# descriptinc/audiotools

Measured on NVIDIA H100. Metric: clips/sec (10s@44.1kHz) log-mel+LUFS pipeline, higher is better.
Workload: dtype f32

## Files before the change

### audiotools_b200/csrc/fft_warp.cuh

```cuda
#pragma once
#include "b2a_common.h"

namespace b2a {
namespace spectral {

__device__ __forceinline__ float2 rot_mi(float2 a) { return make_float2(a.y, -a.x); }

__device__ __forceinline__ float2 cadd(float2 a, float2 b) { return add2(a, b); }
__device__ __forceinline__ float2 csub(float2 a, float2 b) { return add2(a, neg2(b)); }
__device__ __forceinline__ float2 cmul(float2 a, float2 b) {
  return fma2(bcast2(a.x), b, mul2(bcast2(a.y), make_float2(-b.y, b.x)));
}

__device__ __forceinline__ constexpr float cos_pi16(int j) {
  return j == 0 ? 1.0f
       : j == 1 ? 0.98078528040323043f
       : j == 2 ? 0.92387953251128674f
       : j == 3 ? 0.83146961230254524f
       : j == 4 ? 0.70710678118654752f
       : j == 5 ? 0.55557023301960222f
       : j == 6 ? 0.38268343236508977f
       : j == 7 ? 0.19509032201612827f
       : j == 8 ? 0.0f
                : -cos_pi16(16 - j);
}

__device__ __forceinline__ constexpr float cos_pi32(int j) {
  return (j & 1) == 0 ? cos_pi16(j / 2)
       : j == 1 ? 0.99518472667219689f
       : j == 3 ? 0.95694033573220887f
       : j == 5 ? 0.88192126434835503f
       : j == 7 ? 0.77301045336273696f
       : j == 9 ? 0.63439328416364549f
       : j == 11 ? 0.47139673682599764f
       : j == 13 ? 0.29028467725446236f
       : j == 15 ? 0.09801714032956060f
                 : -cos_pi32(32 - j);
}

template <int R, int K>
__device__ __forceinline__ float2 mul_wr(float2 o) {
  constexpr int j = 32 * K / R;
  if constexpr (j == 0) {
    return o;
  } else if constexpr (j == 8) {
    return make_float2(o.y, -o.x);
  } else if constexpr (j == 4) {
    constexpr float h = 0.70710678118654752f;
    return make_float2(h * (o.x + o.y), h * (o.y - o.x));
  } else if constexpr (j == 12) {
    constexpr float h = 0.70710678118654752f;
    return make_float2(h * (o.y - o.x), -h * (o.x + o.y));
  } else {
    constexpr float c = cos_pi16(j);
    constexpr float sn = cos_pi16(j <= 8 ? 8 - j : j - 8);
    return make_float2(fmaf(o.x, c, o.y * sn), fmaf(o.y, c, -o.x * sn));
  }
}

template <int R, int S, bool PRE = false>
struct DFT {
  template <int K>
  static __device__ __forceinline__ void comb(const float2 (&e)[R / 2], const float2 (&o)[R / 2], float2* out) {
    constexpr int j = 32 * K / R;
    if constexpr (R == 2 && PRE) {
      out[K] = e[K];
      out[K + R / 2] = o[K];
    } else if constexpr (j == 0) {
      out[K] = add2(e[K], o[K]);
      out[K + R / 2] = add2(e[K], neg2(o[K]));
    } else if constexpr (j == 8) {
      out[K] = add2(e[K], rot_mi(o[K]));
      out[K + R / 2] = add2(e[K], neg2(rot_mi(o[K])));
    } else if constexpr (j == 4 || j == 12) {
      constexpr float h = 0.70710678118654752f;
      const float2 pq = add2(o[K], rot_mi(o[K]));
      float2 s;
      if constexpr (j == 4) s = fma2(bcast2(h), pq, e[K]);
      else s = fma2(make_float2(h, -h), make_float2(pq.y, pq.x), e[K]);
      out[K] = s;
      out[K + R / 2] = fma2(bcast2(2.0f), e[K], neg2(s));
    } else {
      constexpr float c = cos_pi16(j);
      constexpr float sn = cos_pi16(j <= 8 ? 8 - j : j - 8);
      const float2 s = fma2(o[K], bcast2(c), fma2(rot_mi(o[K]), bcast2(sn), e[K]));
      out[K] = s;
      out[K + R / 2] = fma2(bcast2(2.0f), e[K], neg2(s));
    }
    if constexpr (K + 1 < R / 2) comb<K + 1>(e, o, out);
  }
  static __device__ __forceinline__ void run(const float2* in, float2* out) {
    float2 e[R / 2], o[R / 2];
    DFT<R / 2, 2 * S, PRE>::run(in, e);
    DFT<R / 2, 2 * S, PRE>::run(in + S, o);
    comb<0>(e, o, out);
  }
};
template <int S, bool PRE>
struct DFT<1, S, PRE> {
  static __device__ __forceinline__ void run(const float2* in, float2* out) { out[0] = in[0]; }
};

template <int LOG2N>
struct WPlan {
  static constexpr int N = 1 << LOG2N;
  static constexpr int LPF = N / 32;
  static constexpr int FPW = 32 / LPF;
  static constexpr int R1 = LPF;
  static constexpr int B1 = 32 / R1;
  static constexpr int NWARP = 8;
  static constexpr int G = NWARP * FPW;
  static constexpr int FR = (G >= 16) ? G : (LOG2N == 10 ? 8 : 16);
  static constexpr bool LEAN = (LOG2N == 10);
  static constexpr int NTW = LEAN ? 10 : ((R1 >= 2) ? B1 * (R1 - 1) : 0);
  static constexpr int NUT = LEAN ? 1 : 16;
  static constexpr int XB = ((N + N / 32 + 4 + 3) / 4) * 4 + (N >= 256 ? 128 : 32);
};

__device__ __forceinline__ float fast_sqrt(float v) {
#ifdef B2A_SIM
  return sqrtf(v);
#else
  float r;
  asm("sqrt.approx.ftz.f32 %0, %1;" : "=f"(r) : "f"(v));
  return r;
#endif
}

__device__ __forceinline__ float fast_log2(float v) {
#ifdef B2A_SIM
  return log2f(v);
#else
  float r;
  asm("lg2.approx.f32 %0, %1;" : "=f"(r) : "f"(v));
  return r;
#endif
}

template <int LOG2N, bool PRE0 = false>
__device__ __forceinline__ void warp_fft(float2 (&z)[32], float* xb, const float2* tw, int l) {
  using PL = WPlan<LOG2N>;
  constexpr int LPF = PL::LPF, R1 = PL::R1, B1 = PL::B1;
  {
    float2 o[32];
    DFT<32, 1, PRE0>::run(z, o);
#pragma unroll
    for (int t = 0; t < 32; ++t) z[t] = o[t];
  }
  if constexpr (R1 >= 2) {
#pragma unroll
    for (int t = 0; t < 32; ++t) xb[l * 33 + t] = z[t].x;
    __syncwarp();
#pragma unroll
    for (int m = 0; m < 32; ++m) { const int e = l + LPF * m; z[m].x = xb[e + (e >> 5)]; }
    __syncwarp();
#pragma unroll
    for (int t = 0; t < 32; ++t) xb[l * 33 + t] = z[t].y;
    __syncwarp();
#pragma unroll
    for (int m = 0; m < 32; ++m) { const int e = l + LPF * m; z[m].y = xb[e + (e >> 5)]; }
    __syncwarp();
    if constexpr (PL::LEAN) {
      const float2 w8 = tw[7 * LPF + l], w16 = tw[8 * LPF + l], w24 = tw[9 * LPF + l];
      z[8] = cmul(z[8], w8); z[16] = cmul(z[16], w16); z[24] = cmul(z[24], w24);
#pragma unroll
      for (int b = 1; b < 8; ++b) {
        const float2 wb = tw[(b - 1) * LPF + l];
        z[b] = cmul(z[b], wb);
        z[8 + b] = cmul(cmul(z[8 + b], wb), w8);
        z[16 + b] = cmul(cmul(z[16 + b], wb), w16);
        z[24 + b] = cmul(cmul(z[24 + b], wb), w24);
      }
    }
#pragma unroll
    for (int b = 0; b < B1; ++b) {
      if constexpr (!PL::LEAN) {
#pragma unroll
        for (int t = 1; t < R1; ++t)
          z[b + B1 * t] = cmul(z[b + B1 * t], tw[(b * (R1 - 1) + (t - 1)) * LPF + l]);
      }
      float2 o[R1];
      DFT<R1, B1>::run(&z[b], o);
#pragma unroll
      for (int t = 0; t < R1; ++t) z[b + B1 * t] = o[t];
    }
  }
}

template <int LOG2N, int M>
__device__ __forceinline__ float2 untangle_twiddle(const float2* ut, float2 u0, int l) {
  using PL = WPlan<LOG2N>;
  if constexpr (PL::LEAN) {
    if constexpr (M == 0) {
      return u0;
    } else {
      constexpr float c = cos_pi32(M), sn = cos_pi32(16 - M);
      return fma2(bcast2(u0.x), make_float2(c, -sn), mul2(bcast2(u0.y), make_float2(sn, c)));
    }
  } else {
    return ut[M * PL::LPF + l];
  }
}

template <int LOG2N>
__device__ __forceinline__ float2 untangle_twiddle_m(const float2* ut, float2 u0, int l, int m) {
  switch (m) {
    case 0: return untangle_twiddle<LOG2N, 0>(ut, u0, l);
    case 1: return untangle_twiddle<LOG2N, 1>(ut, u0, l);
    case 2: return untangle_twiddle<LOG2N, 2>(ut, u0, l);
    case 3: return untangle_twiddle<LOG2N, 3>(ut, u0, l);
    case 4: return untangle_twiddle<LOG2N, 4>(ut, u0, l);
    case 5: return untangle_twiddle<LOG2N, 5>(ut, u0, l);
    case 6: return untangle_twiddle<LOG2N, 6>(ut, u0, l);
    case 7: return untangle_twiddle<LOG2N, 7>(ut, u0, l);
    case 8: return untangle_twiddle<LOG2N, 8>(ut, u0, l);
    case 9: return untangle_twiddle<LOG2N, 9>(ut, u0, l);
    case 10: return untangle_twiddle<LOG2N, 10>(ut, u0, l);
    case 11: return untangle_twiddle<LOG2N, 11>(ut, u0, l);
    case 12: return untangle_twiddle<LOG2N, 12>(ut, u0, l);
    case 13: return untangle_twiddle<LOG2N, 13>(ut, u0, l);
    case 14: return untangle_twiddle<LOG2N, 14>(ut, u0, l);
    default: return untangle_twiddle<LOG2N, 15>(ut, u0, l);
  }
}

template <int LOG2N>
__device__ __forceinline__ void untangle(const float2 (&z)[32], const float2* ut, int l, int src_lane, float2 (&a)[16],
                                         float2 (&b)[16], float2& h) {
  const float2 u0 = ut[l];
#pragma unroll
  for (int m = 0; m < 16; ++m) {
    const float2 zk = z[m];
    float2 zn;
    zn.x = __shfl_sync(0xffffffffu, z[31 - m].x, src_lane);
    zn.y = __shfl_sync(0xffffffffu, z[31 - m].y, src_lane);
    if (l == 0) zn = z[(32 - m) & 31];
    const float2 xe = add2(zk, make_float2(zn.x, -zn.y));
    const float2 xo = add2(make_float2(zk.y, -zk.x), make_float2(zn.y, zn.x));
    const float2 w = untangle_twiddle_m<LOG2N>(ut, u0, l, m);
    const float2 xk = fma2(bcast2(w.x), xo, fma2(make_float2(-w.y, w.y), make_float2(xo.y, xo.x), xe));
    const float2 d = fma2(bcast2(2.0f), xe, neg2(xk));
    a[m] = xk;
    b[m] = make_float2(d.x, -d.y);
  }
  h = make_float2(2.0f * z[16].x, -2.0f * z[16].y);
}


template <int LPF>
__device__ __forceinline__ int partner_lane(int lane) {
  return (lane & ~(LPF - 1)) | ((LPF - (lane & (LPF - 1))) & (LPF - 1));
}

template <int LOG2N>
__device__ __forceinline__ void load_frame(const float* fs, const float* win, int hop, float2 (&z)[32], int l) {
  constexpr int LPF = WPlan<LOG2N>::LPF;
  if ((hop & 1) == 0) {
#pragma unroll
    for (int m = 0; m < 16; ++m) {
      const int e0 = l + LPF * m, e1 = e0 + LPF * 16;
      const float2 s0 = *reinterpret_cast<const float2*>(fs + 2 * e0);
      const float2 w0 = *reinterpret_cast<const float2*>(win + 2 * e0);
      const float2 s1 = *reinterpret_cast<const float2*>(fs + 2 * e1);
      const float2 w1 = *reinterpret_cast<const float2*>(win + 2 * e1);
      const float2 a = mul2(s0, w0);
      z[m] = fma2(s1, w1, a);
      z[m + 16] = fma2(neg2(s1), w1, a);
    }
  } else {
#pragma unroll
    for (int m = 0; m < 16; ++m) {
      const int e0 = l + LPF * m, e1 = e0 + LPF * 16;
      const float ax = fs[2 * e0] * win[2 * e0], ay = fs[2 * e0 + 1] * win[2 * e0 + 1];
      const float sx = fs[2 * e1], sy = fs[2 * e1 + 1], wx = win[2 * e1], wy = win[2 * e1 + 1];
      z[m] = make_float2(fmaf(sx, wx, ax), fmaf(sy, wy, ay));
      z[m + 16] = make_float2(fmaf(-sx, wx, ax), fmaf(-sy, wy, ay));
    }
  }
}

template <int LOG2N, int NUT = 16>
__device__ __forceinline__ void warp_fft_tables(float2* tw, float2* ut) {
  using PL = WPlan<LOG2N>;
  constexpr int N = PL::N, LPF = PL::LPF, R1 = PL::R1;
  const int tid = threadIdx.x, nt = blockDim.x;
  for (int i = tid; i < PL::NTW * LPF; i += nt) {
    const int slot = i / LPF, ll = i - slot * LPF;
    int e;
    if constexpr (PL::LEAN) {
      e = ll * (slot < 7 ? slot + 1 : 8 * (slot - 6));
    } else {
      const int b = slot / (R1 > 1 ? R1 - 1 : 1), t = slot - b * (R1 > 1 ? R1 - 1 : 1) + 1;
      e = (ll + LPF * b) * t;
    }
    float sn, cs;
    sincospif(-2.0f * (float)e / (float)N, &sn, &cs);
    tw[i] = make_float2(cs, sn);
  }
  for (int i = tid; i < NUT * LPF; i += nt) {
    const int m = i / LPF, ll = i - m * LPF;
    float sn, cs;
    sincospif(-(float)(ll + LPF * m) / (float)N, &sn, &cs);
    ut[i] = make_float2(cs, sn);
  }
}

}
}
```

### audiotools_b200/csrc/spectral.cu

```cuda
#include "b2a_common.h"
#include "fft_warp.cuh"
#include "grad_internal.h"
#include "spectral_internal.h"

namespace b2a {
namespace spectral {

constexpr int THREADS = 256;
constexpr int E = 16;

template <int LOG2N>
struct Plan {
  static constexpr int N = 1 << LOG2N;
  static constexpr int TPF = N / E;
  static constexpr int G = THREADS / TPF;
  static constexpr int P = (LOG2N + 3) / 4;
  static constexpr int radix(int p) {
    return (p < LOG2N / 4) ? 16 : (1 << (LOG2N % 4));
  }
  static constexpr int ns(int p) { return 1 << (4 * p); }
  static constexpr int slots(int p) { return p == 0 ? 0 : (E / radix(p)) * (radix(p) - 1); }
  static constexpr int slot_off(int p) {
    int o = 0;
    for (int i = 1; i < p; ++i) o += slots(i);
    return o;
  }
  static constexpr int NSLOT = slot_off(P);
  static constexpr int BUF = N + N / 16 + 1;
  static constexpr int MAG = N + 4;
  static constexpr int FR = (G >= 16) ? G : ((LOG2N >= 11) ? 2 * G : ((LOG2N == 10) ? 4 * G : 16));
};

__device__ __forceinline__ void stage_span(const Params& p, float* sp, int row, int tile, int n0, int FR, int ws,
                                           float g) {
  const int tid = threadIdx.x, T = p.T, hop = p.hop, span = p.span;
  const float* xr = p.x + (size_t)row * (size_t)T;
  const int own_lo = n0 * hop;
  const int own_hi = (tile == p.n_tiles - 1) ? T : min(T, (n0 + FR) * hop);
  const bool interior = (ws >= 0) && (ws + span <= T);
  if (interior) {
    const float* src = xr + ws;
    const bool vec = ((((uintptr_t)src) & 15) == 0) && ((span & 3) == 0) &&
                     (!p.y_out || (((uintptr_t)(p.y_out + (size_t)row * T + ws)) & 15) == 0);
    if (vec) {
      for (int i = tid * 4; i < span; i += (int)blockDim.x * 4) {
        float4 v = *reinterpret_cast<const float4*>(src + i);
        if (p.gain) { v.x *= g; v.y *= g; v.z *= g; v.w *= g; }
        *reinterpret_cast<float4*>(sp + i) = v;
        if (p.y_out) {
          const int w = ws + i;
          if (w >= own_lo && w + 3 < own_hi) {
            *reinterpret_cast<float4*>(p.y_out + (size_t)row * T + w) = v;
          } else {
            float vv[4] = {v.x, v.y, v.z, v.w};
#pragma unroll
            for (int e = 0; e < 4; ++e)
              if (w + e >= own_lo && w + e < own_hi) p.y_out[(size_t)row * T + w + e] = vv[e];
          }
        }
      }
    } else {
      for (int i = tid; i < span; i += (int)blockDim.x) {
        float v = __ldg(src + i);
        if (p.gain) v *= g;
        sp[i] = v;
        const int w = ws + i;
        if (p.y_out && w >= own_lo && w < own_hi) p.y_out[(size_t)row * T + w] = v;
      }
    }
  } else {
    for (int i = tid; i < span; i += (int)blockDim.x) {
      const int w = ws + i;
      const int u = src_index(w, T, p.pad, p.right_pad, p.pad_mode);
      float v = (u >= 0) ? __ldg(xr + u) : 0.f;
      if (p.gain) v *= g;
      sp[i] = v;
      if (p.y_out && w >= own_lo && w < own_hi) p.y_out[(size_t)row * T + w] = v;
    }
  }
  if (p.y_out) {
    for (int w = max(own_lo, ws + span) + tid; w < own_hi; w += (int)blockDim.x) {
      float v = __ldg(xr + w);
      if (p.gain) v *= g;
      p.y_out[(size_t)row * T + w] = v;
    }
  }
}

__device__ __forceinline__ void writeback_scaled(const Params& p, const float* sp, int row, int tile, int n0, int FR,
                                                 int ws, float g) {
  const int tid = threadIdx.x, T = p.T, hop = p.hop, span = p.span;
  const int own_lo = n0 * hop;
  const int own_hi = (tile == p.n_tiles - 1) ? T : min(T, (n0 + FR) * hop);
  float* yr = p.y_out + (size_t)row * (size_t)T;
  const int lo = max(own_lo, ws), hi = min(own_hi, ws + span);
  const bool vec = (((lo - ws) & 3) == 0) && ((((uintptr_t)(yr + lo)) & 15) == 0);
  if (vec) {
    const int n4 = (hi - lo) >> 2;
    for (int i = tid; i < n4; i += (int)blockDim.x) {
      float4 v = *reinterpret_cast<const float4*>(sp + (lo - ws) + 4 * i);
      v.x *= g; v.y *= g; v.z *= g; v.w *= g;
      st_stream4(yr + lo + 4 * i, v);
    }
    for (int w = lo + 4 * n4 + tid; w < hi; w += (int)blockDim.x) yr[w] = sp[w - ws] * g;
  } else {
    for (int w = lo + tid; w < hi; w += (int)blockDim.x) yr[w] = sp[w - ws] * g;
  }
  const float* xr = p.x + (size_t)row * (size_t)T;
  for (int w = max(own_lo, ws + span) + tid; w < own_hi; w += (int)blockDim.x) yr[w] = __ldg(xr + w) * g;
}

template <int TPF>
__device__ __forceinline__ void group_sync(int g) {
  if constexpr (TPF >= 64) {
    B2A_BAR_SYNC(1 + g, TPF);
  } else {
    __syncwarp();
  }
}

template <int LOG2N>
__device__ __forceinline__ int buf_phys(int i) { return i + (i >> 4); }

template <int LOG2N, int PASS>
__device__ __forceinline__ void fft_pass(float2 (&v)[E], float2* buf, const float2* tw, int q) {
  using PL = Plan<LOG2N>;
  constexpr int R = PL::radix(PASS), NS = PL::ns(PASS), B = E / R, TPF = PL::TPF;
#pragma unroll
  for (int b = 0; b < B; ++b) {
#pragma unroll
    for (int t = 1; t < R; ++t) {
      float2 w = tw[(PL::slot_off(PASS) + b * (R - 1) + (t - 1)) * TPF + q];
      v[b + B * t] = cmul(v[b + B * t], w);
    }
    float2 out[R];
    DFT<R, B>::run(&v[b], out);
    const int j = q + TPF * b;
    const int k = j & (NS - 1);
    const int base = (j - k) * R + k;
#pragma unroll
    for (int t = 0; t < R; ++t) buf[buf_phys<LOG2N>(base + t * NS)] = out[t];
  }
}

template <int LOG2N>
__global__ void __launch_bounds__(THREADS) spectral_kernel(Params p) {
  using PL = Plan<LOG2N>;
  constexpr int N = PL::N, TPF = PL::TPF, G = PL::G, FR = PL::FR, P = PL::P;
  B2A_DYN_SMEM(smem);
  float* sp = reinterpret_cast<float*>(smem);
  float* win = reinterpret_cast<float*>(smem + p.off_win);
  float2* tw = reinterpret_cast<float2*>(smem + p.off_tw);
  float2* ut = reinterpret_cast<float2*>(smem + p.off_ut);
  float2* bufs = reinterpret_cast<float2*>(smem + p.off_buf);
  float* mags = reinterpret_cast<float*>(smem + p.off_mag);
  float* melt = reinterpret_cast<float*>(smem + p.off_mel);

  const int tid = threadIdx.x;
  const int row = blockIdx.x / p.n_tiles;
  const int tile = blockIdx.x - row * p.n_tiles;
  const int n0 = tile * FR;
  const int hop = p.hop, n_fft = 2 * N;
  const float g = p.gain ? __ldg(p.gain + row / p.rows_per_gain) : 1.0f;
  const int ws = (n0 + p.drop_edge) * hop - N - p.pad;

  for (int i = tid; i < n_fft; i += THREADS) win[i] = __ldg(p.window + i);
  for (int i = tid; i < PL::NSLOT * TPF; i += THREADS) {
    const int slot = i / TPF, q = i - slot * TPF;
    int pass = 1;
#pragma unroll
    for (int pp = 1; pp < P; ++pp)
      if (slot >= PL::slot_off(pp)) pass = pp;
    const int R = PL::radix(pass), NS = PL::ns(pass);
    const int s = slot - PL::slot_off(pass);
    const int b = s / (R - 1), t = s - b * (R - 1) + 1;
    const int k = (q + TPF * b) & (NS - 1);
    float sn, cs;
    sincospif(-2.0f * (float)(k * t) / (float)(NS * R), &sn, &cs);
    tw[i] = make_float2(cs, sn);
  }
  for (int i = tid; i <= N / 2; i += THREADS) {
    float sn, cs;
    sincospif(-(float)i / (float)N, &sn, &cs);
    ut[i] = make_float2(cs, sn);
  }

  stage_span(p, sp, row, tile, n0, FR, ws, g);
  __syncthreads();

  const int grp = tid / TPF, q = tid - grp * TPF;
  float2* buf = bufs + grp * PL::BUF;
  float* mag = mags + grp * PL::MAG;
  const int F = N + 1;

  for (int rd = 0; rd < FR / G; ++rd) {
    const int f = rd * G + grp;
    const int n = n0 + f;
    const bool live = n < p.n_frames;
    const float* fs = sp + f * hop;

    float2 v[E];
    if ((hop & 1) == 0) {
#pragma unroll
      for (int m = 0; m < E; ++m) {
        const int e = q + TPF * m;
        const float2 s2 = *reinterpret_cast<const float2*>(fs + 2 * e);
        const float2 w2 = *reinterpret_cast<const float2*>(win + 2 * e);
        v[m] = make_float2(s2.x * w2.x, s2.y * w2.y);
      }
    } else {
#pragma unroll
      for (int m = 0; m < E; ++m) {
        const int e = q + TPF * m;
        v[m] = make_float2(fs[2 * e] * win[2 * e], fs[2 * e + 1] * win[2 * e + 1]);
      }
    }
    {
      float2 out[E];
      DFT<E, 1>::run(v, out);
#pragma unroll
      for (int t = 0; t < E; ++t) buf[buf_phys<LOG2N>(q * E + t)] = out[t];
    }
    group_sync<TPF>(grp);
    if constexpr (P >= 2) {
#pragma unroll
      for (int m = 0; m < E; ++m) v[m] = buf[buf_phys<LOG2N>(q + TPF * m)];
      group_sync<TPF>(grp);
      fft_pass<LOG2N, 1>(v, buf, tw, q);
      group_sync<TPF>(grp);
    }
    if constexpr (P >= 3) {
#pragma unroll
      for (int m = 0; m < E; ++m) v[m] = buf[buf_phys<LOG2N>(q + TPF * m)];
      group_sync<TPF>(grp);
      fft_pass<LOG2N, 2>(v, buf, tw, q);
      group_sync<TPF>(grp);
    }

    for (int k = q; k <= N / 2; k += TPF) {
      const float2 zk = buf[buf_phys<LOG2N>(k)];
      const float2 zn = buf[buf_phys<LOG2N>((N - k) & (N - 1))];
      const float2 xe = make_float2(0.5f * (zk.x + zn.x), 0.5f * (zk.y - zn.y));
      const float2 xo = make_float2(0.5f * (zk.y + zn.y), 0.5f * (zn.x - zk.x));
      const float2 tt = cmul(ut[k], xo);
      const float2 xk = cadd(xe, tt);
      const float2 d = csub(xe, tt);
      const float2 xnk = make_float2(d.x, -d.y);
      if (p.stft_out && live) {
        float2* o = p.stft_out + (size_t)row * F * p.n_frames + n;
        o[(size_t)k * p.n_frames] = xk;
        o[(size_t)(N - k) * p.n_frames] = xnk;
      }
      mag[k] = sqrtf(fmaf(xk.x, xk.x, xk.y * xk.y));
      mag[N - k] = sqrtf(fmaf(xnk.x, xnk.x, xnk.y * xnk.y));
    }
    group_sync<TPF>(grp);

    if (p.mel_out) {
      for (int m = q; m < p.n_mels; m += TPF) {
        const int lo = __ldg(p.mel_lo + m), hi = __ldg(p.mel_hi + m);
        const float* wrow = p.mel_fb + (size_t)m * F;
        float acc = 0.f;
        for (int k = lo; k < hi; ++k) acc = fmaf(__ldg(wrow + k), mag[k], acc);
        if (p.post == B2A_POST_LOG10) {
          float c = fmaxf(acc, p.post_eps);
          c = (p.post_power == 2.0f) ? c * c : powf(c, p.post_power);
          acc = log10f(c);
        } else if (p.post == B2A_POST_LN) {
          acc = logf(acc + p.post_eps);
        }
        melt[m * (FR + 1) + f] = acc;
      }
    }
    group_sync<TPF>(grp);
  }

  if (p.mel_out) {
    __syncthreads();
    const int nf = min(FR, p.n_frames - n0);
    float* o = p.mel_out + (size_t)row * p.n_mels * p.n_frames + n0;
    for (int i = tid; i < p.n_mels * FR; i += THREADS) {
      const int m = i / FR, f = i - m * FR;
      if (f < nf) o[(size_t)m * p.n_frames + f] = melt[m * (FR + 1) + f];
    }
  }
}

template <int LOG2N>
static int launch(Params& p, void* stream) {
  using PL = Plan<LOG2N>;
  p.span = (PL::FR - 1) * p.hop + p.n_fft;
  p.n_tiles = (p.n_frames + PL::FR - 1) / PL::FR;
  int o = align16(p.span * 4);
  p.off_win = o; o = align16(o + p.n_fft * 4);
  p.off_tw = o; o = align16(o + PL::NSLOT * PL::TPF * 8 + 16);
  p.off_ut = o; o = align16(o + (PL::N / 2 + 1) * 8);
  p.off_buf = o; o = align16(o + PL::G * PL::BUF * 8);
  p.off_mag = o; o = align16(o + PL::G * PL::MAG * 4);
  p.off_mel = o; o = align16(o + (p.mel_out ? p.n_mels * (PL::FR + 1) * 4 : 0));
  p.smem_bytes = o;
  B2A_REQUIRE(o <= 227 * 1024, B2A_E_UNSUPPORTED,
              "spectral: n_fft=%d hop=%d n_mels=%d needs %d bytes of shared memory (> 227 KB)", p.n_fft, p.hop,
              p.n_mels, o);
  B2A_REQUIRE((int64_t)p.rows * p.n_tiles < (int64_t)2147483647, B2A_E_UNSUPPORTED, "spectral: grid too large");
  B2A_CUDA_OK(cudaFuncSetAttribute(spectral_kernel<LOG2N>, cudaFuncAttributeMaxDynamicSharedMemorySize, o));
  B2A_LAUNCH(spectral_kernel<LOG2N>, dim3((unsigned)(p.rows * p.n_tiles)), dim3(THREADS), (size_t)o, stream, p);
  B2A_CUDA_OK(cudaGetLastError());
  return B2A_OK;
}



#ifdef B2A_K1_PROBE
__device__ unsigned long long* g_k1_probe;
#define K1_PROBE_TILES 64
#define K1_STAMP(k)                                                                                   \
  do {                                                                                                \
    if (g_k1_probe && lane == 0 && it_probe < K1_PROBE_TILES)                                         \
      g_k1_probe[(((size_t)blockIdx.x * 8 + warp) * K1_PROBE_TILES + it_probe) * 11 + (k)] = clock64(); \
  } while (0)
#else
#define K1_STAMP(k) do { } while (0)
#endif

template <int LOG2N, int MODE>
__global__ void __launch_bounds__(256, 2) spectral_warp_kernel(Params p) {
  using PL = WPlan<LOG2N>;
  constexpr bool STAGED = (MODE == 1), DIRECT = (MODE == 2);
  constexpr int N = PL::N, LPF = PL::LPF, FPW = PL::FPW, G = PL::G, FR = PL::FR;
  static_assert(FR == G && FR % 8 == 0, "one round per tile: the |X| slot of a frame is its index in the tile");
  B2A_DYN_SMEM(smem);
  float* sp = reinterpret_cast<float*>(smem);
  float* win = reinterpret_cast<float*>(smem + p.off_win);
  float2* tw = reinterpret_cast<float2*>(smem + p.off_tw);
  float2* ut = reinterpret_cast<float2*>(smem + p.off_ut);
  float* xbs = reinterpret_cast<float*>(smem + p.off_buf);
  float* mpk = reinterpret_cast<float*>(smem + p.off_mpk);
  int4* mseg = reinterpret_cast<int4*>(smem + p.off_mseg);

  const int tid = threadIdx.x, lane = tid & 31, warp = tid >> 5;
  const int hop = p.hop, n_fft = 2 * N, F = N + 1;
  const int l = lane & (LPF - 1);
  const int fw = lane / LPF;
  const int total_tiles = p.rows * p.n_tiles;

  int t = blockIdx.x;
  __shared__ __align__(8) unsigned long long s_bar;
  if (tid == 0) mbar_init(&s_bar, 1);
  __syncthreads();
  bool by_tma;
  unsigned tma_parity = 0;
  {
    const int row = t / p.n_tiles, tile = t - row * p.n_tiles;
    by_tma = stage_span_async(p, sp, row,
                              (tile * FR + p.drop_edge) * hop + p.origin + (p.row_origin ? __ldg(p.row_origin + row) : 0),
                              &s_bar);
  }
  for (int i = tid; i < n_fft; i += 256) win[i] = 0.5f * __ldg(p.window + i);
  for (int i = tid; i < G * p.xb_stride; i += 256) xbs[i] = 0.f;
  warp_fft_tables<LOG2N, PL::NUT>(tw, ut);
  const bool packed = p.mel_out && p.mel_packed_len > 0;
  __shared__ int s_clamp;
  if (packed) {
    for (int m = tid; m < p.n_mels; m += 256) {
      const int lo4 = __ldg(p.mel_lo + m) & ~3;
      int n4 = (((__ldg(p.mel_hi + m) + 3) & ~3) - lo4) >> 2;
      mseg[m] = make_int4(0, lo4, n4 < 0 ? 0 : n4, 0);
    }
    __syncthreads();
    if (tid == 0) {
      int run = 0, reach = 0;
      for (int w = 0; w < 8; ++w)
        for (int i = 0; 4 * (w + 8 * i) < p.n_mels; ++i) {
          int mx = 0;
          for (int j = 0; j < 4; ++j) { const int m = 4 * (w + 8 * i) + j; if (m < p.n_mels) mx = max(mx, mseg[m].z); }
          mx = (mx + 1) & ~1;
          for (int j = 0; j < 4; ++j) {
            const int m = 4 * (w + 8 * i) + j;
            if (m < p.n_mels) { mseg[m].x = run; mseg[m].w = mx; run += mx; reach = max(reach, mseg[m].y + 4 * mx); }
          }
        }
      s_clamp = reach > PL::XB;
    }
    __syncthreads();
    for (int m = warp; m < p.n_mels; m += 8) {
      const int4 sg = mseg[m];
      const float* wrow = p.mel_fb + (size_t)m * F;
      for (int i = lane; i < 4 * sg.w; i += 32) {
        const int k = sg.y + i;
        mpk[4 * sg.x + i] = (i < 4 * sg.z && k < F) ? __ldg(wrow + k) : 0.f;
      }
    }
  }

  float* xb = xbs + (warp * FPW + fw) * p.xb_stride;
  const int src_lane = partner_lane<LPF>(lane);

#ifdef B2A_K1_PROBE
  int it_probe = 0;
#endif
  bool first = true;
#pragma unroll 1
  for (; t < total_tiles; t += gridDim.x) {
    const int row = t / p.n_tiles, tile = t - row * p.n_tiles;
    const int n0 = tile * FR;
    const int ws = (n0 + p.drop_edge) * hop + p.origin + (p.row_origin ? __ldg(p.row_origin + row) : 0);
    const float g = p.gain ? __ldg(p.gain + row / p.rows_per_gain) : 1.0f;
    const float ga = fabsf(g);
    K1_STAMP(0);
    if (by_tma) { mbar_wait(&s_bar, tma_parity); tma_parity ^= 1u; }
    K1_STAMP(1);
#ifdef B2A_SIM
    __syncthreads();
#else
    if (!by_tma || first) __syncthreads();
#endif
    first = false;
    K1_STAMP(2);
    if (p.y_out) writeback_scaled(p, sp, row, tile, n0, FR, ws, g);
    K1_STAMP(3);

#pragma unroll 1
    for (int rd = 0; rd < FR / G; ++rd) {
      const int f = rd * G + warp * FPW + fw;
      const int n = n0 + f;
      const bool live = n < p.n_frames;
      const float* fs = sp + f * hop;

      float2 z[32];
      load_frame<LOG2N>(fs, win, hop, z, l);
      K1_STAMP(4);
      if (rd == FR / G - 1) {
        __syncthreads();
        const int tn = t + gridDim.x;
        by_tma = false;
        if (tn < total_tiles) {
          const int rown = tn / p.n_tiles, tilen = tn - rown * p.n_tiles;
          by_tma = stage_span_async(
              p, sp, rown, (tilen * FR + p.drop_edge) * hop + p.origin + (p.row_origin ? __ldg(p.row_origin + rown) : 0),
              &s_bar);
        }
      }
      K1_STAMP(5);
      warp_fft<LOG2N, true>(z, xb, tw, l);

      const float2 u0 = ut[l];
      float2* so = (DIRECT && p.stft_out) ? p.stft_out + (size_t)row * F * p.n_frames + n : nullptr;
#pragma unroll
      for (int m = 0; m < 16; ++m) {
        const float2 zk = z[m];
        float2 zn;
        zn.x = __shfl_sync(0xffffffffu, z[31 - m].x, src_lane);
        zn.y = __shfl_sync(0xffffffffu, z[31 - m].y, src_lane);
        if (l == 0) zn = z[(32 - m) & 31];
        const int k = l + LPF * m;
        const float2 xe = add2(zk, make_float2(zn.x, -zn.y));
        const float2 xo = add2(make_float2(zk.y, -zk.x), make_float2(zn.y, zn.x));
        const float2 w = untangle_twiddle_m<LOG2N>(ut, u0, l, m);
        const float2 xk = fma2(bcast2(w.x), xo, fma2(make_float2(-w.y, w.y), make_float2(xo.y, xo.x), xe));
        const float2 d = fma2(bcast2(2.0f), xe, neg2(xk));
        if constexpr (STAGED) {
          float2* xc = reinterpret_cast<float2*>(xb);
          xc[k] = make_float2(g * xk.x, g * xk.y);
          xc[N - k] = make_float2(g * d.x, -g * d.y);
        } else {
          if constexpr (DIRECT) {
            if (so && live) {
              so[(size_t)k * p.n_frames] = make_float2(g * xk.x, g * xk.y);
              so[(size_t)(N - k) * p.n_frames] = make_float2(g * d.x, -g * d.y);
            }
          }
          xb[k] = fast_sqrt(fmaf(xk.x, xk.x, xk.y * xk.y));
          xb[N - k] = fast_sqrt(fmaf(d.x, d.x, d.y * d.y));
        }
      }
      if (l == 0) {
        const float2 zh = make_float2(2.0f * z[16].x, 2.0f * z[16].y);
        if constexpr (STAGED) {
          reinterpret_cast<float2*>(xb)[N / 2] = make_float2(g * zh.x, -g * zh.y);
        } else {
          if constexpr (DIRECT) {
            if (so && live) so[(size_t)(N / 2) * p.n_frames] = make_float2(g * zh.x, -g * zh.y);
          }
          xb[N / 2] = fast_sqrt(fmaf(zh.x, zh.x, zh.y * zh.y));
          xb[N + 1] = 0.f; xb[N + 2] = 0.f; xb[N + 3] = 0.f;
        }
      }
      __syncwarp();

    }
    K1_STAMP(6);

    const int nf = min(FR, p.n_frames - n0);
    float* mo = p.mel_out ? p.mel_out + (size_t)row * p.n_mels * p.n_frames + n0 : nullptr;
    if (p.mel_out) {
      __syncthreads();
      K1_STAMP(7);
      const int fl = lane & 7, jq = lane >> 3;
      const float lscale = p.post_power * 0.30102999566398120f;
      if (packed) {
        const float4* mpk4 = reinterpret_cast<const float4*>(mpk);
        for (int fc = 0; fc < FR; fc += 8) {
          const int f = fc + fl;
          const float* xf = xbs + f * p.xb_stride;
          if (!s_clamp) {
            for (int mm = 4 * warp + jq; mm < p.n_mels; mm += 32) {
              const int4 sg = mseg[mm];
              const float4* w4 = mpk4 + sg.x;
              const float4* v4 = reinterpret_cast<const float4*>(xf + sg.y);
              float2 a01 = make_float2(0.f, 0.f), a23 = a01;
              for (int it = 0; it < sg.w; it += 2) {
                const float4 wa = w4[it], wb = w4[it + 1], va = v4[it], vb = v4[it + 1];
                a01 = fma2(make_float2(wa.x, wa.y), make_float2(va.x, va.y), a01);
                a23 = fma2(make_float2(wb.x, wb.y), make_float2(vb.x, vb.y), a23);
                a01 = fma2(make_float2(wa.z, wa.w), make_float2(va.z, va.w), a01);
                a23 = fma2(make_float2(wb.z, wb.w), make_float2(vb.z, vb.w), a23);
              }
              float acc = ((a01.x + a01.y) + (a23.x + a23.y)) * ga;
              if (p.post == B2A_POST_LOG10) acc = lscale * fast_log2(fmaxf(acc, p.post_eps));
              else if (p.post == B2A_POST_LN) acc = logf(acc + p.post_eps);
              if (f < nf) mo[(size_t)mm * p.n_frames + f] = acc;
            }
          } else {
            const int lim = PL::XB - 4;
            for (int mm = 4 * warp + jq; mm < p.n_mels; mm += 32) {
              const int4 sg = mseg[mm];
              const float4* w4 = mpk4 + sg.x;
              float a0 = 0.f, a1 = 0.f;
              for (int it = 0; it < sg.w; ++it) {
                const float4 w = w4[it];
                const float4 v = *reinterpret_cast<const float4*>(xf + min(sg.y + 4 * it, lim));
                a0 = fmaf(w.x, v.x, a0); a1 = fmaf(w.y, v.y, a1);
                a0 = fmaf(w.z, v.z, a0); a1 = fmaf(w.w, v.w, a1);
              }
              float acc = (a0 + a1) * ga;
              if (p.post == B2A_POST_LOG10) acc = lscale * fast_log2(fmaxf(acc, p.post_eps));
              else if (p.post == B2A_POST_LN) acc = logf(acc + p.post_eps);
              if (f < nf) mo[(size_t)mm * p.n_frames + f] = acc;
            }
          }
        }
      } else {
        for (int fc = 0; fc < FR; fc += 8) {
          const int f = fc + fl;
          const float* xf = xbs + f * p.xb_stride;
          for (int mm = 4 * warp + jq; mm < p.n_mels; mm += 32) {
            float acc = mel_band(p.mel_fb, p.mel_lo, p.mel_hi, F, mm, xf) * ga;
            if (p.post == B2A_POST_LOG10) acc = lscale * fast_log2(fmaxf(acc, p.post_eps));
            else if (p.post == B2A_POST_LN) acc = logf(acc + p.post_eps);
            if (f < nf) mo[(size_t)mm * p.n_frames + f] = acc;
          }
        }
      }
    }

    K1_STAMP(8);
    if constexpr (STAGED) {
      __syncthreads();
      const int nf = min(FR, p.n_frames - n0);
      float2* o = p.stft_out + (size_t)row * F * p.n_frames + n0;
      for (int i = tid; i < F * FR; i += 256) {
        const int k = i / FR, f = i - k * FR;
        if (f < nf) o[(size_t)k * p.n_frames + f] = reinterpret_cast<const float2*>(xbs + f * p.xb_stride)[k];
      }
    }
    K1_STAMP(9);
    K1_STAMP(10);
#ifdef B2A_K1_PROBE
    ++it_probe;
#endif
  }
}

#ifdef B2A_K1_PROBE
static int g_k1_last[3];
#endif

template <int LOG2N>
static int launch_warp(Params& p, void* stream) {
  using PL = WPlan<LOG2N>;
  p.span = (PL::FR - 1) * p.hop + p.n_fft;
  p.n_tiles = (p.n_frames + PL::FR - 1) / PL::FR;
  int o = align16(p.span * 4);
  p.off_win = o; o = align16(o + p.n_fft * 4);
  p.off_tw = o; o = align16(o + PL::NTW * PL::LPF * 8 + 16);
  p.off_ut = o; o = align16(o + PL::NUT * PL::LPF * 8);
  p.xb_stride = PL::XB;
  p.stage_stft = 0;
  if (p.stft_out && !p.mel_out) {
    const int wide = ((2 * PL::N + 4 + 3) / 4) * 4;
    if (wide >= PL::XB && o + PL::G * wide * 4 + 64 <= 112 * 1024) { p.xb_stride = wide; p.stage_stft = 1; }
  }
  p.off_buf = o; o = align16(o + PL::G * p.xb_stride * 4);
  p.off_mag = o;
  p.off_mel = o;
  const int base = o;
  p.off_mpk = o; p.off_mseg = o;
  if (p.mel_out && p.mel_packed_len > 0) {
    p.off_mpk = o; o = align16(o + p.mel_packed_len * 4);
    p.off_mseg = o; o = align16(o + p.n_mels * 16);
    if (o > 227 * 1024) { o = base; p.mel_packed_len = 0; }
  }
  p.smem_bytes = o;
  B2A_REQUIRE(o <= 227 * 1024, B2A_E_UNSUPPORTED,
              "spectral: n_fft=%d hop=%d n_mels=%d needs %d bytes of shared memory (> 227 KB)", p.n_fft, p.hop,
              p.n_mels, o);
  const int64_t total = (int64_t)p.rows * p.n_tiles;
  B2A_REQUIRE(total < (int64_t)2147483647, B2A_E_UNSUPPORTED, "spectral: too many tiles");
  auto kern = p.stage_stft ? spectral_warp_kernel<LOG2N, 1>
                           : (p.stft_out ? spectral_warp_kernel<LOG2N, 2> : spectral_warp_kernel<LOG2N, 0>);
  B2A_CUDA_OK(cudaFuncSetAttribute(kern, cudaFuncAttributeMaxDynamicSharedMemorySize, o));
  int64_t grid;
  const int rc = persistent_grid(kern, o, total, &grid);
  if (rc != B2A_OK) return rc;
#ifdef B2A_K1_PROBE
  if (LOG2N == 10 && !p.stft_out) {
    B2A_CUDA_OK(cudaOccupancyMaxActiveBlocksPerMultiprocessor(&g_k1_last[0], kern, 256, (size_t)o));
    g_k1_last[1] = (int)grid; g_k1_last[2] = o;
  }
#endif
  B2A_LAUNCH(kern, dim3((unsigned)grid), dim3(256), (size_t)o, stream, p);
  B2A_CUDA_OK(cudaGetLastError());
  return B2A_OK;
}

int frames_fft(const float* x, int rows, int T, int n_fft, int hop, const float* window, int origin,
               const int32_t* row_origin, int pad_mode, int n_frames, float2* out, void* stream) {
  Params p;
  memset(&p, 0, sizeof(p));
  p.x = x; p.window = window; p.stft_out = out;
  p.rows = rows; p.T = T; p.n_fft = n_fft; p.hop = hop; p.pad_mode = pad_mode; p.n_frames = n_frames;
  p.rows_per_gain = 1; p.center = 0; p.origin = origin; p.row_origin = row_origin;
  switch (n_fft) {
    case 64: return launch_warp<5>(p, stream);
    case 128: return launch_warp<6>(p, stream);
    case 256: return launch_warp<7>(p, stream);
    case 512: return launch_warp<8>(p, stream);
    case 1024: return launch_warp<9>(p, stream);
    case 2048: return launch_warp<10>(p, stream);
  }
  return b2a::fail(B2A_E_UNSUPPORTED, "frames_fft: block size %d", n_fft);
}

int check_framing(const char* who, int64_t T, int n_fft, int hop, int pad, int right_pad, int pad_mode, int drop_edge,
                  int64_t* n_frames) {
  B2A_REQUIRE(pad >= 0 && right_pad >= 0 && drop_edge >= 0, B2A_E_INVALID, "%s: negative padding", who);
  B2A_REQUIRE(pad_mode >= 0 && pad_mode <= 2, B2A_E_UNSUPPORTED, "%s: pad mode %d", who, pad_mode);
  const int64_t Lp = T + 2 * (int64_t)pad + right_pad;
  B2A_REQUIRE(n_fft / 2 < Lp, B2A_E_INVALID, "%s: n_fft/2 (%d) must be < padded length (%lld)", who, n_fft / 2,
              (long long)Lp);
  B2A_REQUIRE(pad_mode != B2A_PAD_REFLECT || (pad + right_pad) < T || (pad + right_pad) == 0, B2A_E_INVALID,
              "%s: reflect padding (%d) must be < signal length (%lld)", who, pad + right_pad, (long long)T);
  *n_frames = b2a_stft_num_frames(T, n_fft, hop, pad, right_pad, drop_edge);
  B2A_REQUIRE(*n_frames >= 1, B2A_E_INVALID, "%s: no frames", who);
  return B2A_OK;
}

}
}

extern "C" int64_t b2a_stft_num_frames(int64_t T, int n_fft, int hop, int pad, int right_pad, int drop_edge) {
  if (T < 1 || n_fft < 2 || hop < 1 || pad < 0 || right_pad < 0 || drop_edge < 0) return -1;
  int64_t n = 1 + (T + 2 * (int64_t)pad + right_pad - (n_fft & 1)) / hop - 2 * (int64_t)drop_edge;
  return n;
}

extern "C" int b2a_stft_route(int n_fft, int hop, int inverse) {
  if (n_fft < 2 || hop < 1 || (inverse && hop > n_fft)) return B2A_ROUTE_NONE;
  if ((n_fft & (n_fft - 1)) == 0) {
    if (n_fft >= (inverse ? 64 : 32) && n_fft <= (inverse ? 2048 : 4096)) return B2A_ROUTE_FFT;
    if (n_fft >= 4096 && n_fft <= 32768) return B2A_ROUTE_LARGE;
  }
  return n_fft <= 8192 ? B2A_ROUTE_DENSE : B2A_ROUTE_NONE;
}

static int spectral_fft(const float* x, int64_t rows, int64_t T, int n_fft, int hop, const float* window, int pad,
                        int right_pad, int pad_mode, int drop_edge, const float* gain, int rows_per_gain, float* y_out,
                        const float* mel_fb, const int32_t* mel_lo, const int32_t* mel_hi, int n_mels,
                        int mel_packed_len, int post, float post_eps, float post_power, float* mel_out,
                        float* stft_out, void* stream) {
  using namespace b2a::spectral;
  B2A_REQUIRE(x && window, B2A_E_INVALID, "spectral: null x/window");
  B2A_REQUIRE(mel_out || stft_out, B2A_E_INVALID, "spectral: neither mel_out nor stft_out requested");
  B2A_REQUIRE(rows >= 1 && T >= 1, B2A_E_INVALID, "spectral: empty input");
  B2A_REQUIRE(T < (int64_t)1 << 30, B2A_E_UNSUPPORTED, "spectral: rows longer than 2^30 samples");
  B2A_REQUIRE(n_fft >= 32 && n_fft <= 4096 && (n_fft & (n_fft - 1)) == 0, B2A_E_UNSUPPORTED,
              "spectral: window_length must be a power of two in [32, 4096] (got %d)", n_fft);
  B2A_REQUIRE(hop >= 1, B2A_E_INVALID, "spectral: hop_length must be >= 1");
  int64_t nfr;
  const int rc = check_framing("spectral", T, n_fft, hop, pad, right_pad, pad_mode, drop_edge, &nfr);
  if (rc != B2A_OK) return rc;
  B2A_REQUIRE(!y_out || (pad == 0 && right_pad == 0 && drop_edge == 0), B2A_E_UNSUPPORTED,
              "spectral: y_out needs pad == right_pad == drop_edge == 0");
  B2A_REQUIRE(!gain || rows_per_gain >= 1, B2A_E_INVALID, "spectral: rows_per_gain");
  B2A_REQUIRE(!mel_out || (mel_fb && mel_lo && mel_hi && n_mels >= 1), B2A_E_INVALID, "spectral: mel arguments");
  B2A_REQUIRE(post >= 0 && post <= 2, B2A_E_INVALID, "spectral: post-op %d", post);
  Params p;
  memset(&p, 0, sizeof(p));
  p.x = x; p.window = window; p.gain = gain; p.y_out = y_out;
  p.mel_fb = mel_fb; p.mel_lo = mel_lo; p.mel_hi = mel_hi; p.mel_out = mel_out;
  p.stft_out = reinterpret_cast<float2*>(stft_out);
  p.rows = (int)rows; p.T = (int)T; p.n_fft = n_fft; p.hop = hop; p.pad = pad; p.right_pad = right_pad;
  p.pad_mode = pad_mode; p.drop_edge = drop_edge; p.n_frames = (int)nfr; p.n_mels = n_mels;
  p.mel_packed_len = (mel_out && mel_packed_len > 0) ? mel_packed_len : 0;
  p.center = 1; p.origin = -(n_fft / 2) - pad; p.row_origin = nullptr;
  p.rows_per_gain = gain ? rows_per_gain : 1; p.post = post; p.post_eps = post_eps; p.post_power = post_power;
  switch (n_fft) {
    case 32: return launch<4>(p, stream);
    case 64: return launch_warp<5>(p, stream);
    case 128: return launch_warp<6>(p, stream);
    case 256: return launch_warp<7>(p, stream);
    case 512: return launch_warp<8>(p, stream);
    case 1024: return launch_warp<9>(p, stream);
    case 2048: return launch_warp<10>(p, stream);
    case 4096: return launch<11>(p, stream);
  }
  return b2a::fail(B2A_E_UNSUPPORTED, "spectral: n_fft %d", n_fft);
}

extern "C" size_t b2a_spectral_workspace_bytes(int64_t rows, int64_t T, int n_fft, int hop, int pad, int right_pad,
                                                int drop_edge, int stft_scratch, int scaled_scratch) {
  const int r = b2a_stft_route(n_fft, hop, 0);
  const int64_t nfr = b2a_stft_num_frames(T, n_fft, hop, pad, right_pad, drop_edge);
  if (rows < 1 || nfr < 1 || r == B2A_ROUTE_NONE || r == B2A_ROUTE_FFT) return 0;
  size_t bytes = 0;
  if (stft_scratch) bytes += (size_t)rows * (size_t)(n_fft / 2 + 1) * (size_t)nfr * 2 * sizeof(float);
  if (scaled_scratch) bytes += (size_t)rows * (size_t)T * sizeof(float);
  return bytes;
}

static int spectral_materialised(int route, const float* x, int64_t rows, int64_t T, int n_fft, int hop,
                                 const float* window, const float* matrix, int pad, int right_pad, int pad_mode,
                                 int drop_edge, const float* gain, int rows_per_gain, float* y_out,
                                 const float* mel_fb, const int32_t* mel_lo, const int32_t* mel_hi, int n_mels,
                                 int post, float post_eps, float post_power, float* mel_out, float* stft_out,
                                 void* ws, size_t ws_bytes, void* stream) {
  B2A_REQUIRE(mel_out || stft_out, B2A_E_INVALID, "spectral: neither mel_out nor stft_out requested");
  int64_t nfr;
  int rc = b2a::spectral::check_framing(route == B2A_ROUTE_LARGE ? "stft_large" : "stft_dense", T, n_fft, hop, pad,
                                        right_pad, pad_mode, drop_edge, &nfr);
  if (rc != B2A_OK) return rc;
  const size_t need = b2a_spectral_workspace_bytes(rows, T, n_fft, hop, pad, right_pad, drop_edge, !stft_out,
                                                   gain && !y_out);
  B2A_REQUIRE(ws_bytes >= need && (ws || need == 0), B2A_E_INVALID, "spectral: workspace too small");
  B2A_REQUIRE(((uintptr_t)ws & 7) == 0, B2A_E_INVALID, "spectral: workspace must be 8-byte aligned");
  const int F = n_fft / 2 + 1;
  char* scratch = static_cast<char*>(ws);
  float* stft = stft_out;
  if (!stft) {
    stft = reinterpret_cast<float*>(scratch);
    scratch += (size_t)rows * F * (size_t)nfr * 2 * sizeof(float);
  }
  if (gain) {
    B2A_REQUIRE(rows_per_gain >= 1 && rows % rows_per_gain == 0, B2A_E_INVALID, "spectral: rows_per_gain");
    float* scaled = y_out ? y_out : reinterpret_cast<float*>(scratch);
    rc = b2a_gain_f32(x, scaled, rows / rows_per_gain, rows_per_gain * T, gain, stream);
    if (rc != B2A_OK) return rc;
    x = scaled;
  }
  rc = route == B2A_ROUTE_LARGE
           ? b2a::large::stft(x, rows, T, n_fft, hop, window, pad, right_pad, pad_mode, drop_edge, stft, stream)
           : b2a::dft::stft(x, rows, T, n_fft, hop, matrix, pad, right_pad, pad_mode, drop_edge, stft, stream);
  if (rc != B2A_OK || !mel_out) return rc;
  return b2a::dft::mel_from_stft(stft, rows, F, nfr, mel_fb, mel_lo, mel_hi, n_mels, post, post_eps, post_power,
                                 mel_out, stream);
}

extern "C" int b2a_spectral_f32(const float* x, int64_t rows, int64_t T, int n_fft, int hop, const float* window,
                                const float* matrix, int pad, int right_pad, int pad_mode, int drop_edge,
                                const float* gain, int rows_per_gain, float* y_out, const float* mel_fb,
                                const int32_t* mel_lo, const int32_t* mel_hi, int n_mels, int mel_packed_len, int post,
                                float post_eps, float post_power, float* mel_out, float* stft_out, void* ws,
                                size_t ws_bytes, void* stream) {
  const int route = b2a_stft_route(n_fft, hop, 0);
  if (route == B2A_ROUTE_FFT)
    return spectral_fft(x, rows, T, n_fft, hop, window, pad, right_pad, pad_mode, drop_edge, gain, rows_per_gain, y_out,
                        mel_fb, mel_lo, mel_hi, n_mels, mel_packed_len, post, post_eps, post_power, mel_out, stft_out,
                        stream);
  if (route == B2A_ROUTE_LARGE || route == B2A_ROUTE_DENSE)
    return spectral_materialised(route, x, rows, T, n_fft, hop, window, matrix, pad, right_pad, pad_mode, drop_edge,
                                 gain, rows_per_gain, y_out, mel_fb, mel_lo, mel_hi, n_mels, post, post_eps, post_power,
                                 mel_out, stft_out, ws, ws_bytes, stream);
  return b2a::fail(B2A_E_UNSUPPORTED,
                   "spectral: n_fft=%d hop=%d (hop >= 1; powers of two up to 32768, any other length up to 8192)",
                   n_fft, hop);
}

extern "C" int b2a_spectral_tc_enable(int on) {
  if (on == 0) return 0;
  return b2a::fail(B2A_E_UNSUPPORTED,
                   "spectral_tc_enable: the tensor-core spectral kernel was removed; the FP32 kernel runs every launch");
}

#ifdef B2A_K1_PROBE
extern "C" int b2a_k1_probe_set(void* buf) {
  B2A_CUDA_OK(cudaMemcpyToSymbol(b2a::spectral::g_k1_probe, &buf, sizeof(buf)));
  return B2A_OK;
}
extern "C" int b2a_k1_probe_tiles() { return K1_PROBE_TILES; }
extern "C" void b2a_k1_probe_last(int* out) {
  for (int i = 0; i < 3; ++i) out[i] = b2a::spectral::g_k1_last[i];
}
#endif
```

Measured before the change: 101,500.

## Vectorize warp FFT exchange, pair window table, precompute untangle twiddles

The warp FFT transpose now writes rows with a 36-float stride using float4 stores instead of scalar stores with a 33-stride. The window is stored interleaved in shared memory so one float4 load fetches both halves' coefficients. In lean plans the untangle twiddle table is expanded to all 16 rows at setup, so the per-frame recomputation becomes a table lookup. The mel inner loop is pinned to no unrolling. The costs are more shared memory for the tables, possible bank conflicts on the strided-36 reads, and an extra block sync at setup.

```diff
diff --git a/audiotools_b200/csrc/fft_warp.cuh b/audiotools_b200/csrc/fft_warp.cuh
--- a/audiotools_b200/csrc/fft_warp.cuh
+++ b/audiotools_b200/csrc/fft_warp.cuh
@@ -137,7 +137,7 @@
 #endif
 }
 
-template <int LOG2N, bool PRE0 = false>
+template <int LOG2N, bool PRE0 = false, int XS = 33>
 __device__ __forceinline__ void warp_fft(float2 (&z)[32], float* xb, const float2* tw, int l) {
   using PL = WPlan<LOG2N>;
   constexpr int LPF = PL::LPF, R1 = PL::R1, B1 = PL::B1;
@@ -148,17 +148,30 @@
     for (int t = 0; t < 32; ++t) z[t] = o[t];
   }
   if constexpr (R1 >= 2) {
-#pragma unroll
-    for (int t = 0; t < 32; ++t) xb[l * 33 + t] = z[t].x;
+    static_assert(XS == 33 || XS == 36, "exchange row stride");
+    if constexpr (XS == 36) {
+#pragma unroll
+      for (int t = 0; t < 32; t += 4)
+        *reinterpret_cast<float4*>(xb + l * XS + t) = make_float4(z[t].x, z[t + 1].x, z[t + 2].x, z[t + 3].x);
+    } else {
+#pragma unroll
+      for (int t = 0; t < 32; ++t) xb[l * XS + t] = z[t].x;
+    }
     __syncwarp();
 #pragma unroll
-    for (int m = 0; m < 32; ++m) { const int e = l + LPF * m; z[m].x = xb[e + (e >> 5)]; }
+    for (int m = 0; m < 32; ++m) { const int e = l + LPF * m; z[m].x = xb[(e >> 5) * XS + (e & 31)]; }
     __syncwarp();
-#pragma unroll
-    for (int t = 0; t < 32; ++t) xb[l * 33 + t] = z[t].y;
+    if constexpr (XS == 36) {
+#pragma unroll
+      for (int t = 0; t < 32; t += 4)
+        *reinterpret_cast<float4*>(xb + l * XS + t) = make_float4(z[t].y, z[t + 1].y, z[t + 2].y, z[t + 3].y);
+    } else {
+#pragma unroll
+      for (int t = 0; t < 32; ++t) xb[l * XS + t] = z[t].y;
+    }
     __syncwarp();
 #pragma unroll
-    for (int m = 0; m < 32; ++m) { const int e = l + LPF * m; z[m].y = xb[e + (e >> 5)]; }
+    for (int m = 0; m < 32; ++m) { const int e = l + LPF * m; z[m].y = xb[(e >> 5) * XS + (e & 31)]; }
     __syncwarp();
     if constexpr (PL::LEAN) {
       const float2 w8 = tw[7 * LPF + l], w16 = tw[8 * LPF + l], w24 = tw[9 * LPF + l];
@@ -252,7 +265,7 @@
   return (lane & ~(LPF - 1)) | ((LPF - (lane & (LPF - 1))) & (LPF - 1));
 }
 
-template <int LOG2N>
+template <int LOG2N, bool PAIRED = false>
 __device__ __forceinline__ void load_frame(const float* fs, const float* win, int hop, float2 (&z)[32], int l) {
   constexpr int LPF = WPlan<LOG2N>::LPF;
   if ((hop & 1) == 0) {
@@ -260,9 +273,16 @@
     for (int m = 0; m < 16; ++m) {
       const int e0 = l + LPF * m, e1 = e0 + LPF * 16;
       const float2 s0 = *reinterpret_cast<const float2*>(fs + 2 * e0);
-      const float2 w0 = *reinterpret_cast<const float2*>(win + 2 * e0);
-      const float2 s1 = *reinterpret_cast<const float2*>(fs + 2 * e1);
-      const float2 w1 = *reinterpret_cast<const float2*>(win + 2 * e1);
+      float2 w0, s1, w1;
+      if constexpr (PAIRED) {
+        const float4 w = reinterpret_cast<const float4*>(win)[e0];
+        w0 = make_float2(w.x, w.y); w1 = make_float2(w.z, w.w);
+        s1 = *reinterpret_cast<const float2*>(fs + 2 * e1);
+      } else {
+        w0 = *reinterpret_cast<const float2*>(win + 2 * e0);
+        s1 = *reinterpret_cast<const float2*>(fs + 2 * e1);
+        w1 = *reinterpret_cast<const float2*>(win + 2 * e1);
+      }
       const float2 a = mul2(s0, w0);
       z[m] = fma2(s1, w1, a);
       z[m + 16] = fma2(neg2(s1), w1, a);
@@ -271,12 +291,27 @@
 #pragma unroll
     for (int m = 0; m < 16; ++m) {
       const int e0 = l + LPF * m, e1 = e0 + LPF * 16;
-      const float ax = fs[2 * e0] * win[2 * e0], ay = fs[2 * e0 + 1] * win[2 * e0 + 1];
-      const float sx = fs[2 * e1], sy = fs[2 * e1 + 1], wx = win[2 * e1], wy = win[2 * e1 + 1];
+      float ax, ay, sx, sy, wx, wy;
+      if constexpr (PAIRED) {
+        const float4 w = reinterpret_cast<const float4*>(win)[e0];
+        ax = fs[2 * e0] * w.x; ay = fs[2 * e0 + 1] * w.y;
+        sx = fs[2 * e1]; sy = fs[2 * e1 + 1]; wx = w.z; wy = w.w;
+      } else {
+        ax = fs[2 * e0] * win[2 * e0]; ay = fs[2 * e0 + 1] * win[2 * e0 + 1];
+        sx = fs[2 * e1]; sy = fs[2 * e1 + 1]; wx = win[2 * e1]; wy = win[2 * e1 + 1];
+      }
       z[m] = make_float2(fmaf(sx, wx, ax), fmaf(sy, wy, ay));
       z[m + 16] = make_float2(fmaf(-sx, wx, ax), fmaf(-sy, wy, ay));
     }
   }
+}
+
+template <int LOG2N>
+__device__ __forceinline__ void pair_window(float* win, const float* w, float scale) {
+  constexpr int N = WPlan<LOG2N>::N;
+  for (int e = threadIdx.x; e < N / 2; e += blockDim.x)
+    reinterpret_cast<float4*>(win)[e] = make_float4(scale * __ldg(w + 2 * e), scale * __ldg(w + 2 * e + 1),
+                                                    scale * __ldg(w + 2 * e + N), scale * __ldg(w + 2 * e + N + 1));
 }
 
 template <int LOG2N, int NUT = 16>
@@ -305,5 +340,16 @@
   }
 }
 
-}
-}
+template <int LOG2N>
+__device__ __forceinline__ void expand_untangle_table(float2* ut) {
+  constexpr int LPF = WPlan<LOG2N>::LPF;
+  if constexpr (WPlan<LOG2N>::LEAN) {
+    for (int i = LPF + threadIdx.x; i < 16 * LPF; i += blockDim.x) {
+      const int m = i / LPF, ll = i - m * LPF;
+      ut[i] = untangle_twiddle_m<LOG2N>(ut, ut[ll], ll, m);
+    }
+  }
+}
+
+}
+}
diff --git a/audiotools_b200/csrc/spectral.cu b/audiotools_b200/csrc/spectral.cu
--- a/audiotools_b200/csrc/spectral.cu
+++ b/audiotools_b200/csrc/spectral.cu
@@ -329,6 +329,7 @@
   constexpr bool STAGED = (MODE == 1), DIRECT = (MODE == 2);
   constexpr int N = PL::N, LPF = PL::LPF, FPW = PL::FPW, G = PL::G, FR = PL::FR;
   static_assert(FR == G && FR % 8 == 0, "one round per tile: the |X| slot of a frame is its index in the tile");
+  static_assert(LPF * 36 <= PL::XB, "the exchange plane of warp_fft<..., 36> fits a frame slot");
   B2A_DYN_SMEM(smem);
   float* sp = reinterpret_cast<float*>(smem);
   float* win = reinterpret_cast<float*>(smem + p.off_win);
@@ -339,7 +340,7 @@
   int4* mseg = reinterpret_cast<int4*>(smem + p.off_mseg);
 
   const int tid = threadIdx.x, lane = tid & 31, warp = tid >> 5;
-  const int hop = p.hop, n_fft = 2 * N, F = N + 1;
+  const int hop = p.hop, F = N + 1;
   const int l = lane & (LPF - 1);
   const int fw = lane / LPF;
   const int total_tiles = p.rows * p.n_tiles;
@@ -356,9 +357,13 @@
                               (tile * FR + p.drop_edge) * hop + p.origin + (p.row_origin ? __ldg(p.row_origin + row) : 0),
                               &s_bar);
   }
-  for (int i = tid; i < n_fft; i += 256) win[i] = 0.5f * __ldg(p.window + i);
+  pair_window<LOG2N>(win, p.window, 0.5f);
   for (int i = tid; i < G * p.xb_stride; i += 256) xbs[i] = 0.f;
   warp_fft_tables<LOG2N, PL::NUT>(tw, ut);
+  if constexpr (PL::LEAN) {
+    __syncthreads();
+    expand_untangle_table<LOG2N>(ut);
+  }
   const bool packed = p.mel_out && p.mel_packed_len > 0;
   __shared__ int s_clamp;
   if (packed) {
@@ -428,7 +433,7 @@
       const float* fs = sp + f * hop;
 
       float2 z[32];
-      load_frame<LOG2N>(fs, win, hop, z, l);
+      load_frame<LOG2N, true>(fs, win, hop, z, l);
       K1_STAMP(4);
       if (rd == FR / G - 1) {
         __syncthreads();
@@ -442,9 +447,8 @@
         }
       }
       K1_STAMP(5);
-      warp_fft<LOG2N, true>(z, xb, tw, l);
-
-      const float2 u0 = ut[l];
+      warp_fft<LOG2N, true, 36>(z, xb, tw, l);
+
       float2* so = (DIRECT && p.stft_out) ? p.stft_out + (size_t)row * F * p.n_frames + n : nullptr;
 #pragma unroll
       for (int m = 0; m < 16; ++m) {
@@ -456,7 +460,7 @@
         const int k = l + LPF * m;
         const float2 xe = add2(zk, make_float2(zn.x, -zn.y));
         const float2 xo = add2(make_float2(zk.y, -zk.x), make_float2(zn.y, zn.x));
-        const float2 w = untangle_twiddle_m<LOG2N>(ut, u0, l, m);
+        const float2 w = ut[m * LPF + l];
         const float2 xk = fma2(bcast2(w.x), xo, fma2(make_float2(-w.y, w.y), make_float2(xo.y, xo.x), xe));
         const float2 d = fma2(bcast2(2.0f), xe, neg2(xk));
         if constexpr (STAGED) {
@@ -509,6 +513,7 @@
               const float4* w4 = mpk4 + sg.x;
               const float4* v4 = reinterpret_cast<const float4*>(xf + sg.y);
               float2 a01 = make_float2(0.f, 0.f), a23 = a01;
+#pragma unroll 1
               for (int it = 0; it < sg.w; it += 2) {
                 const float4 wa = w4[it], wb = w4[it + 1], va = v4[it], vb = v4[it + 1];
                 a01 = fma2(make_float2(wa.x, wa.y), make_float2(va.x, va.y), a01);
@@ -584,7 +589,7 @@
   int o = align16(p.span * 4);
   p.off_win = o; o = align16(o + p.n_fft * 4);
   p.off_tw = o; o = align16(o + PL::NTW * PL::LPF * 8 + 16);
-  p.off_ut = o; o = align16(o + PL::NUT * PL::LPF * 8);
+  p.off_ut = o; o = align16(o + 16 * PL::LPF * 8);
   p.xb_stride = PL::XB;
   p.stage_stft = 0;
   if (p.stft_out && !p.mel_out) {
```

New measurement: 105,800 (median of 6 runs). 1.04x the previous value.
